# A2R-Lab/indy7-mpc

Measured on AMD Instinct MI355X. Metric: SQP-MPC solves/sec (Indy7 6-DOF, N=32), higher is better.
Workload: dtype f64

## Files before the change

indy7_mpc_amd/csrc/i7m_admm.h:

```cpp
#pragma once

#include "i7m_kernels.h"

namespace i7m {

struct AdmmCfg {
  double rho0, sigma, alpha, eps_abs, eps_rel, adapt_tol;
  int max_iter, check, scaling, gap, adapt_interval, pad;
};

struct AdmmArgs {
  SolveParams P;
  AdmmCfg A;
  const double* lin;
  const double* cost;
  const double* qpd;
  const double* xu;
  const double* xs;
  const int* active;
  double* sol;
  double *sx, *sz, *sy, *sq, *srho;
  double *Pq, *Pd, *I, *qs, *ls, *D, *E, *Dt, *Et, *R, *w;
  double* cs;
  int* iters;
  int* status;
  int sqp_iter;
  int b0;
  int ablate;
  const double* abase;
  long abytes;
};

constexpr int ADMM_FSTRIDE = 19;
constexpr int ADMM_SCALE_WPE = 2;
constexpr int ADMM_FACTOR_WPE = 2;
constexpr int ADM_REC = 300, REC_J = 180;
__device__ __forceinline__ int adm_lw(int i) { return i < 16 ? 2 * ((i + 2) / 2) : 18; }
__device__ __forceinline__ int adm_lrow(int i) {
  const int h = i >> 1;
  return i < 16 ? 2 * h * (h + 1) + (i & 1) * (2 * h + 2) : 144 + 18 * (i - 16);
}
__device__ __forceinline__ int adm_lrec(int i, int j) { return adm_lrow(i) + j; }
constexpr unsigned A5_OOB = 0x7ff00000u;
__device__ __forceinline__ __amdgpu_buffer_rsrc_t a4_rsrc(const void* base, long bytes) {
  const unsigned long long u = (unsigned long long)base;
  const unsigned lo = __builtin_amdgcn_readfirstlane((unsigned)u), hi = __builtin_amdgcn_readfirstlane((unsigned)(u >> 32));
  const int nb = __builtin_amdgcn_readfirstlane((int)bytes);
  return __builtin_amdgcn_make_buffer_rsrc((void*)(((unsigned long long)hi << 32) | lo), (short)0, nb, 0x00020000);
}
__device__ __forceinline__ void adm_stage_J(double* sJ, const double* Jc, int l) {
  for (int e = l; e < 216; e += 64) {
    const int i = e / 18, j = e - 18 * i;
    double v;
    if (i < 6) v = j == i ? Jc[i] : (j == 6 + i ? Jc[6 + i] : 0.0);
    else v = Jc[12 + 18 * (i - 6) + j];
    sJ[e] = v;
  }
}

template <int n>
__device__ __forceinline__ double adm_dot2(double init, const double* a, int sa, const double* b, int sb) {
  double av[n], bv[n];
#pragma unroll
  for (int i = 0; i < n; ++i) {
    av[i] = a[sa * i];
    bv[i] = b[sb * i];
  }
  double acc = init;
#pragma unroll
  for (int i = 0; i < n; ++i) acc += av[i] * bv[i];
  return acc;
}

template <int W>
__device__ __forceinline__ double adm_max(double v) {
#pragma unroll
  for (int off = W / 2; off >= 1; off >>= 1) v = fmax(v, __shfl_xor(v, off, W));
  return v;
}
template <int W>
__device__ __forceinline__ double adm_sum(double v) {
#pragma unroll
  for (int off = W / 2; off >= 1; off >>= 1) v += __shfl_xor(v, off, W);
  return v;
}
__device__ __forceinline__ double adm_wave_max(double v) { return adm_max<64>(v); }
__device__ __forceinline__ double adm_wave_sum(double v) { return adm_sum<64>(v); }
__device__ __forceinline__ double adm_limit(double v) { return v < 1e-4 ? 1.0 : (v > 1e4 ? 1e4 : v); }

__device__ __forceinline__ double adm_jk(const double* L, double dt, int i, int j) {
  if (i < 6) return j == i ? 1.0 : (j == 6 + i ? dt : 0.0);
  const int r = i - 6;
  return j < 6 ? L[6 * r + j] : (j < 12 ? L[36 + 6 * r + j - 6] : L[72 + 6 * r + j - 12]);
}

#define ADM_CHK_LOADS_FIRST()                          \
  do {                                                 \
    __builtin_amdgcn_sched_group_barrier(0x020, 24, 0); \
    __builtin_amdgcn_sched_group_barrier(0x002, 96, 0); \
  } while (0)

__device__ inline bool adm_check(const AdmmArgs& a, int N, int T, int m, double c, double rho, const double* x,
                                 const double* z, const double* y, const double* qs, const double* ls, const double* D,
                                 const double* E, const double* Jb, const double* Ib, const double* Pq, const double* Pd,
                                 double* rho_est, int l, double es = 1.0) {
  constexpr int W = 16;
  double pr = 0.0, zn = 0.0, an = 0.0, pri = 0.0, pn = 0.0;
  double dr = 0.0, qn = 0.0, atn = 0.0, pxn = 0.0, dua = 0.0, dn = 0.0, xPx = 0.0, qx = 0.0, sc = 0.0;
  for (int r = l; r < m; r += W) {
    const int k = r / 12, i = r - 12 * k;
    const int kk = k > 0 ? k - 1 : 0, iq = i < 6 ? i : 0, iv = i < 6 ? 0 : i - 6;
    const double* G = Jb + ADM_REC * kk;
    const double* xk = x + 18 * kk;
    const double* Gr = G + 12 + 18 * iv;
    const double ib = Ib[r], xr = x[18 * k + i], er = E[r], zr = z[r], yr = y[r], lr = ls[r];
    const double ga = G[iq], gb = G[6 + iq], xa = xk[iq], xb = xk[6 + iq];
    double gv[18], xv[18];
#pragma unroll
    for (int j = 0; j < 18; ++j) {
      gv[j] = Gr[j];
      xv[j] = xk[j];
    }
    ADM_CHK_LOADS_FIRST();
    double aq = 0.0, av = 0.0;
    aq += ga * xa;
    aq += gb * xb;
#pragma unroll
    for (int j = 0; j < 18; ++j) av += gv[j] * xv[j];
    const double acc = i < 6 ? aq : av;
    const double ax = k == 0 ? ib * xr : acc + ib * xr;
    const double ei = 1.0 / er;
    pr = fmax(pr, fabs(ei * (ax - zr)));
    zn = fmax(zn, fabs(ei * zr));
    an = fmax(an, fabs(ei * ax));
    pri = fmax(pri, fabs(ax - zr));
    pn = fmax(pn, fmax(fabs(zr), fabs(ax)));
    sc += lr * fmax(yr, 0.0) + lr * fmin(yr, 0.0);
  }
  for (int e = l; e < T; e += W) {
    const int k = e / 18, j = e - 18 * k;
    const int jq = j < 12 ? j : 0, jc = j < 6 ? j : 0, kc = k < N - 1 ? k : 0;
    const int jy = j < 6 ? j : (j < 12 ? j - 6 : 0);
    const double* G = Jb + ADM_REC * kc;
    const double* yk = y + 12 * (k < N - 1 ? k + 1 : 0);
    const double xe = x[e], de = D[e], qe = qs[e], pde = Pd[e], ibj = Ib[12 * k + jq], yj = y[12 * k + jq];
    const double gq = G[jq], yq = yk[jy];
    double pq[6], xq[6], gv[6], yv[6];
#pragma unroll
    for (int t = 0; t < 6; ++t) {
      pq[t] = Pq[36 * k + 6 * jc + t];
      xq[t] = x[18 * k + t];
      gv[t] = G[12 + 18 * t + j];
      yv[t] = yk[6 + t];
    }
    ADM_CHK_LOADS_FIRST();
    double pa = 0.0;
#pragma unroll
    for (int t = 0; t < 6; ++t) pa += pq[t] * xq[t];
    const double px = j < 6 ? pa : pde * xe;
    const double at0 = j < 12 ? ibj * yj : 0.0;
    double at1 = j < 12 ? at0 + gq * yq : at0;
#pragma unroll
    for (int t = 0; t < 6; ++t) at1 += gv[t] * yv[t];
    const double aty = k < N - 1 ? at1 : at0;
    const double di = 1.0 / de;
    dr = fmax(dr, fabs(di * ((qe + px) + aty)));
    qn = fmax(qn, fabs(di * qe));
    atn = fmax(atn, fabs(di * aty));
    pxn = fmax(pxn, fabs(di * px));
    dua = fmax(dua, fabs(qe + px + aty));
    dn = fmax(dn, fmax(fabs(qe), fmax(fabs(aty), fabs(px))));
    xPx += xe * px;
    qx += qe * xe;
  }
  pr = adm_max<W>(pr); zn = adm_max<W>(zn); an = adm_max<W>(an); pri = adm_max<W>(pri); pn = adm_max<W>(pn);
  dr = adm_max<W>(dr); qn = adm_max<W>(qn); atn = adm_max<W>(atn); pxn = adm_max<W>(pxn);
  dua = adm_max<W>(dua); dn = adm_max<W>(dn);
  xPx = adm_sum<W>(xPx); qx = adm_sum<W>(qx); sc = adm_sum<W>(sc);
  const double cinv = 1.0 / c;
  {
    const double p = pri / (pn + 1e-30), d = dua / (dn + 1e-30);
    double rn = rho * sqrt(p / (d + 1e-30));
    *rho_est = fmin(fmax(rn, 1e-6), 1e6);
  }
  dr *= cinv;
  const double ea = es * a.A.eps_abs, er = es * a.A.eps_rel;
  if (!(pr < ea + er * fmax(zn, an))) return false;
  if (!(dr < ea + er * cinv * fmax(qn, fmax(atn, pxn)))) return false;
  if (a.A.gap) {
    xPx *= cinv; qx *= cinv; sc *= cinv;
    const double gp = xPx + qx + sc;
    if (!(fabs(gp) < ea + er * fmax(fabs(xPx), fmax(fabs(qx), fabs(sc))))) return false;
  }
  return true;
}

__device__ __forceinline__ double adm_pq(const double* w, int i, int j) { return w[6] * (w[i] * w[j]); }
template <int CT>
__device__ __forceinline__ double adm_scale(const AdmmArgs& a, int b, int N, int T, int m, const double* LIN,
                                            const double* CO, const double* QD, const double* X, double* qold,
                                            double* Pq, double* Pd, double* Jb, double* Ib, double* qs, double* ls,
                                            double* D, double* E, double* sD, double* sE, double* sDt, double* sRM, int l) {
  constexpr int RT = 2 * CT / 3;
  const double dt = a.P.dt;
  double qv[CT], etv[RT], dtv[CT <= 9 ? CT : 1];
#pragma unroll
  for (int t = 0; t < CT; ++t) {
    const int e = l + 64 * t;
    qv[t] = 0.0;
    if (e < T) {
      sD[e] = 1.0;
      qv[t] = qold[e];
    }
  }
#pragma unroll
  for (int t = 0; t < RT; ++t)
    if (l + 64 * t < m) sE[l + 64 * t] = 1.0;
  wave_sync_fence();
  double c = 1.0;
  auto pcol = [&](const double* Cp, int k, int j, double dj) {
    const double* w = Cp + COST_STRIDE * k;
    const int jq = j < 6 ? j : 0;
    double mq = 0.0;
#pragma unroll
    for (int i = 0; i < 6; ++i) mq = fmax(mq, fabs(adm_pq(w, i, jq)) * (sD[18 * k + i] * dj) * c);
    const double pd = j < 12 ? w[7] : w[8];
    return j < 6 ? mq : fabs(pd) * (dj * dj) * c;
  };
  constexpr bool REG = CT <= 9;
  const int ks = l >> 1, hs = l & 1;
  const bool sv = REG && ks < N - 1;
  double av[REG ? 3 : 1][REG ? 18 : 1];
  if constexpr (REG) {
    const double* L = LIN + LIN_STRIDE * (sv ? ks : 0);
#pragma unroll
    for (int r = 0; r < 3; ++r)
#pragma unroll
      for (int j = 0; j < 18; ++j) {
        const int jb = j < 6 ? j : (j < 12 ? 30 + j : 60 + j);
        av[r][j] = sv ? L[jb + 6 * (3 * hs + r)] : 0.0;
      }
  }
#ifdef I7M_DIAG
  const int ss_p = a.ablate >= 300000 ? a.ablate - 300000 : -1;
  const bool ss_on = ss_p >= 0 && blockIdx.x == 0;
  unsigned long long ss_t[8] = {0, 0, 0, 0, 0, 0, 0, 0};
#endif
#define AS_STAMP(i) I7M_STAMP(ss_t, i, ss_on && pass == ss_p)
  for (int pass = 0; pass < a.A.scaling; ++pass) {
    AS_STAMP(0);
    const double* Lp = LIN;
    const double* Cp = CO;
    int lp = l;
    asm volatile("" : "+v"(lp));
    if constexpr (REG) {
      double cm[18];
#pragma unroll
      for (int j = 0; j < 18; ++j) cm[j] = 0.0;
      const int kq = sv ? ks : 0;
#pragma unroll
      for (int r = 0; r < 3; ++r) {
        const double er = sE[12 * (kq + 1) + 6 + 3 * hs + r];
        double rm = 0.0;
#pragma unroll
        for (int j = 0; j < 18; ++j) {
          const double pv = er * fabs(av[r][j]) * sD[18 * kq + j];
          rm = fmax(rm, pv);
          cm[j] = fmax(cm[j], pv);
        }
        if (sv) sRM[12 * (kq + 1) + 6 + 3 * hs + r] = rm;
      }
#pragma unroll
      for (int j = 0; j < 18; ++j) {
        const long long u = __double_as_longlong(cm[j]);
        const int lo = __builtin_amdgcn_update_dpp(0, (int)u, 0xB1, 0xf, 0xf, true);
// ... 349 lines not shown
```

indy7_mpc_amd/csrc/i7m_admm_iter.h:

```cpp
#pragma once

#include "i7m_admm.h"

namespace i7m {

constexpr int A5_LREC = 316, A5_LJ = 196;
__device__ __forceinline__ int a5_lrow(int i) {
  const int g = i >> 2;
  return i < 16 ? 8 * g * (g + 1) + 4 * (g + 1) * (i - 4 * g) : 160 + 18 * (i - 16);
}

constexpr int A5_RI = 10;
constexpr int A5_VI = 3;
constexpr int A5_VP = 42;
constexpr int A5_RP = A5_LREC / 2;
template <int n>
__device__ __forceinline__ double a4_bc(double v) {
  return __builtin_amdgcn_update_dpp(0.0, v, 0x150 + n, 0xf, 0xf, false);
}
__device__ __forceinline__ double a4_dpp32(double v, int ctrl_is_shl) {
  const long long u = __double_as_longlong(v);
  int lo = (int)u, hi = (int)(u >> 32);
  if (ctrl_is_shl) {
    lo = __builtin_amdgcn_update_dpp(lo, lo, 0x106, 0xf, 0xf, false);
// ... 111 lines not shown
  return {lo, b16, b17};
}
__device__ __forceinline__ A4Vec a4_ltmul(const A4CL& L, const A4CT& C, const A4Vec& v) {
  double lo = a4_dot16<2>(v.lo, C.Lt);
  lo = __fma_rn(L.Lc16, v.h16, lo);
  lo = __fma_rn(L.Lc17, v.h17, lo);
  return {lo, __fma_rn(L.d76, v.h17, __dmul_rn(L.d66, v.h16)), __dmul_rn(L.d77, v.h17)};
}
__device__ __forceinline__ A4Vec a4_jtmul(const A4CJ& C, double u, A4Vec init) {
  const double us = a4_shr6(u);
  const double lo = __dadd_rn(__fma_rn(C.Jd, us, init.lo), a4_dot6(u, C.Jt));
  return {lo, __dadd_rn(init.h16, a4_dot6(u, C.J16)), __dadd_rn(init.h17, a4_dot6(u, C.J17))};
}
__device__ __forceinline__ double a4_jmul(const A4CR& C, int c, const A4Vec& v) {
  double a = a4_dot16(v.lo, C.Jr);
  a = __fma_rn(C.Jr[16], v.h16, a);
  a = __fma_rn(C.Jr[17], v.h17, a);
  const double sp = __fma_rn(C.Jq1, a4_shl6(v.lo), __dmul_rn(C.Jq0, v.lo));
  return c < 6 ? sp : a;
}

typedef unsigned int a4u2 __attribute__((ext_vector_type(2)));
__device__ __forceinline__ double a5_ld(__amdgpu_buffer_rsrc_t r, unsigned off) {
  return __builtin_bit_cast(double, __builtin_amdgcn_raw_buffer_load_b64(r, off, 0, 0));
}
__device__ __forceinline__ void a5_st(double v, __amdgpu_buffer_rsrc_t r, unsigned off) {
  __builtin_amdgcn_raw_buffer_store_b64(__builtin_bit_cast(a4u2, v), r, off, 0, 0);
}
__device__ __forceinline__ unsigned a5_dma_off(int t) { return 1024u * (unsigned)(t & 3); }
__device__ __forceinline__ void a5_dma(__amdgpu_buffer_rsrc_t r, unsigned lds, const unsigned (&ro)[A5_RI], unsigned so,
                                       const unsigned (&vo)[A5_VI]) {
  unsigned keep;
  asm volatile(
      "s_mov_b32 %0, m0\n\t"
      "s_mov_b32 m0, %1\n\t"
      "s_nop 0\n\t"
      "buffer_load_dwordx4 %2, %15, %16 offen lds\n\t"
      "buffer_load_dwordx4 %3, %15, %16 offen offset:1024 lds\n\t"
      "buffer_load_dwordx4 %4, %15, %16 offen offset:2048 lds\n\t"
      "buffer_load_dwordx4 %5, %15, %16 offen offset:3072 lds\n\t"
      "s_add_u32 m0, m0, 0x1000\n\ts_nop 0\n\t"
      "buffer_load_dwordx4 %6, %15, %16 offen lds\n\t"
      "buffer_load_dwordx4 %7, %15, %16 offen offset:1024 lds\n\t"
      "buffer_load_dwordx4 %8, %15, %16 offen offset:2048 lds\n\t"
      "buffer_load_dwordx4 %9, %15, %16 offen offset:3072 lds\n\t"
      "s_add_u32 m0, m0, 0x1000\n\ts_nop 0\n\t"
      "buffer_load_dwordx4 %10, %15, %16 offen lds\n\t"
      "buffer_load_dwordx4 %11, %15, %16 offen offset:1024 lds\n\t"
      "buffer_load_dwordx4 %12, %15, 0 offen offset:2048 lds\n\t"
      "buffer_load_dwordx4 %13, %15, 0 offen offset:3072 lds\n\t"
      "s_add_u32 m0, m0, 0x1000\n\ts_nop 0\n\t"
      "buffer_load_dwordx4 %14, %15, 0 offen lds\n\t"
      "s_mov_b32 m0, %0"
      : "=&s"(keep)
      : "s"(__builtin_amdgcn_readfirstlane(lds)), "v"(ro[0]), "v"(ro[1]), "v"(ro[2]), "v"(ro[3]), "v"(ro[4]), "v"(ro[5]), "v"(ro[6]), "v"(ro[7]),
        "v"(ro[8]), "v"(ro[9]), "v"(vo[0]), "v"(vo[1]), "v"(vo[2]), "s"(r), "s"(__builtin_amdgcn_readfirstlane(so))
      : "memory");
}
__device__ __forceinline__ void a5_wait() { asm volatile("s_waitcnt vmcnt(13)" ::: "memory"); }
__device__ __forceinline__ void a5_dma2(__amdgpu_buffer_rsrc_t r, unsigned lds, const unsigned (&ro)[5], unsigned so,
                                        const unsigned (&vo)[2]) {
  unsigned keep;
  asm volatile(
      "s_mov_b32 %0, m0\n\t"
      "s_mov_b32 m0, %1\n\t"
      "s_nop 0\n\t"
      "buffer_load_dwordx4 %2, %9, %10 offen lds\n\t"
      "buffer_load_dwordx4 %3, %9, %10 offen offset:1024 lds\n\t"
      "buffer_load_dwordx4 %4, %9, %10 offen offset:2048 lds\n\t"
      "buffer_load_dwordx4 %5, %9, %10 offen offset:3072 lds\n\t"
      "s_add_u32 m0, m0, 0x1000\n\ts_nop 0\n\t"
      "buffer_load_dwordx4 %6, %9, %10 offen lds\n\t"
      "buffer_load_dwordx4 %7, %9, 0 offen offset:1024 lds\n\t"
      "buffer_load_dwordx4 %8, %9, 0 offen offset:2048 lds\n\t"
      "s_mov_b32 m0, %0"
      : "=&s"(keep)
      : "s"(__builtin_amdgcn_readfirstlane(lds)), "v"(ro[0]), "v"(ro[1]), "v"(ro[2]), "v"(ro[3]), "v"(ro[4]),
        "v"(vo[0]), "v"(vo[1]), "s"(r), "s"(__builtin_amdgcn_readfirstlane(so))
      : "memory");
}
__device__ __forceinline__ void a5_wait2() { asm volatile("s_waitcnt vmcnt(7)" ::: "memory"); }
__device__ __forceinline__ void a5_drain() { asm volatile("s_waitcnt vmcnt(0)" ::: "memory"); }

__device__ __forceinline__ bool a4_check(const AdmmArgs& a, int N, int T, int m, long bq, double c_cost, double rho,
                                         int c, double* rho_est, double es = 1.0) {
  return adm_check(a, N, T, m, c_cost, rho, a.sx + bq * T, a.sz + bq * m, a.sy + bq * m, a.qs + bq * T, a.ls + bq * m,
                   a.D + bq * T, a.E + bq * m, a.R + bq * N * ADM_REC + REC_J, a.I + bq * m, a.Pq + bq * N * 36,
                   a.Pd + bq * T, rho_est, c, es);
}
__device__ __forceinline__ int a4_closing_status(const AdmmArgs& a, int N, int T, int m, long bq, double c_cost,
                                                 double rho, int c, bool solved) {
  auto test = [&](double es) {
    double rest = rho;
    return a4_check(a, N, T, m, bq, c_cost, rho, c, &rest, es);
  };
  const bool last_checked = a.A.check && a.A.max_iter % a.A.check == 0;
  const bool exact = last_checked ? false : test(1.0);
  const bool approx = exact ? false : test(10.0);
  return solved ? 1 : (exact ? 1 : (approx ? 2 : 0));
}
__device__ __forceinline__ void a4_finish(const AdmmArgs& a, long b, bool lead, double rho, bool solved, int done_it,
                                          int status) {
  if (lead) {
    a.srho[b] = rho;
    if (a.iters) a.iters[b * 8 + a.sqp_iter] = solved ? done_it : a.A.max_iter;
    if (a.status) a.status[b * 8 + a.sqp_iter] = status;
  }
}
__device__ __forceinline__ void a4_solution(const AdmmArgs& a, long b, const double* x, int e0, int stride) {
  const int T = a.P.T;
  const double* D = a.D + b * T;
  double* sol = a.sol + b * T;
  for (int e = e0; e < T; e += stride) sol[e] = D[e] * x[e];
}

struct A5Stamps {
#ifdef I7M_DIAG
  unsigned long long t[9] = {0, 0, 0, 0, 0, 0, 0, 0, 0};
  int it, s;
  bool on = false;
  __device__ __forceinline__ explicit A5Stamps(int ablate)
      : it(ablate >= 100000 && ablate < 200000 && blockIdx.x == 0 ? (ablate - 100000) / 100 : -1), s(ablate % 100) {}
  __device__ __forceinline__ void step(int i, int st) { on = i == it && st == s; }
  __device__ __forceinline__ void write(int ablate, int layout) const {
    if (it >= 0) tl_write_stamps(t, 9, ablate, layout);
  }
#else
  __device__ __forceinline__ explicit A5Stamps(int) {}
  __device__ __forceinline__ void step(int, int) {}
  __device__ __forceinline__ void write(int, int) const {}
#endif
};
#define A5_STAMP(st, i) I7M_STAMP((st).t, i, (st).on)

struct A4K {
  int c;
  bool lo12;
  double rv, ri, sg, al, al1;
};
struct A4Op {
  double v0, v1, z1, y1, l1, ib1;
  double2 hv0, hv1;
};
struct A4Co {
  A4CJ J;
  A4CL L;
  A4CT T;
  A4CR Jr;
  const double* R;
};
struct A4Carry {
  A4Vec hc;
  double tk, ibk;
  double b0z, b0y, b0l, b0i, nx0;
  double2 nx0h;
};
struct A4New {
  double zn, yn, xn, xn16, xn17;
};
__device__ __forceinline__ double a4_t(const A4K& K, double z, double y) {
  return __dmul_rn(K.rv, __dsub_rn(z, __dmul_rn(K.ri, y)));
}
__device__ __forceinline__ void a4_coef_begin(A4Co& C, const double* R, int c) {
  C.R = R;
  a4_ldj(C.J, R, c);
  a4_ldl(C.L, R, R + a5_lrow(c), c);
}
template <int SB>
__device__ __forceinline__ A4Vec a4_llt(A4Co& C, const A4Vec& r, bool jr, int c, A5Stamps& st) {
  A5_STAMP(st, SB);
  a4_ldt(C.T, C.R, c);
  const A4Vec y = a4_lmul(C.L, r);
  A5_STAMP(st, SB + 1);
  if (jr) a4_ldr(C.Jr, C.R, c);
  const A4Vec o = a4_ltmul(C.L, C.T, y);
  A5_STAMP(st, SB + 2);
  return o;
}
template <int SB, class Put>
__device__ __forceinline__ void a4_forward(const A4K& K, const A4Op& o, A4Co& C, A4Carry& S, A5Stamps& st, Put&& put) {
  const double t1 = a4_t(K, o.z1, o.y1);
  const double init = K.lo12 ? __dmul_rn(S.ibk, S.tk) : 0.0;
  A4Vec r = a4_jtmul(C.J, t1, A4Vec{init, 0.0, 0.0});
  r.lo = __dadd_rn(__dsub_rn(__dmul_rn(K.sg, o.v0), o.v1), r.lo);
  r.h16 = __dadd_rn(__dsub_rn(__dmul_rn(K.sg, o.hv0.x), o.hv1.x), r.h16);
  r.h17 = __dadd_rn(__dsub_rn(__dmul_rn(K.sg, o.hv0.y), o.hv1.y), r.h17);
  const double rc = __dsub_rn(r.lo, __dmul_rn(__dmul_rn(K.rv, S.ibk), S.hc.lo));
  r.lo = K.lo12 ? rc : r.lo;
  const A4Vec h = a4_llt<SB>(C, r, true, K.c, st);
  put(h);
  A5_STAMP(st, SB + 3);
  S.hc.lo = a4_jmul(C.Jr, K.c, h);
  S.tk = t1;
  S.ibk = o.ib1;
  A5_STAMP(st, SB + 4);
}
template <int SB>
__device__ __forceinline__ void a4_forward_last(const A4K& K, const A4Op& o, A4Co& C, A4Carry& S, A5Stamps& st) {
  A4Vec r{K.lo12 ? __dmul_rn(S.ibk, S.tk) : 0.0, 0.0, 0.0};
  r.lo = __dadd_rn(__dsub_rn(__dmul_rn(K.sg, o.v0), o.v1), r.lo);
  r.lo = __dsub_rn(r.lo, __dmul_rn(__dmul_rn(K.rv, S.ibk), S.hc.lo));
  r.lo = K.lo12 ? r.lo : 0.0;
  S.hc = a4_llt<SB>(C, r, false, K.c, st);
}
__device__ __forceinline__ A4New a4_relax(const A4K& K, double zt, double z, double y, double l, const A4Vec& xt, double x,
                                          double x16, double x17) {
  const double zr = __dadd_rn(__dmul_rn(K.al, zt), __dmul_rn(K.al1, z));
  double zn = __dadd_rn(zr, __dmul_rn(K.ri, y));
  zn = fmin(fmax(zn, l), l);
  const double yn = __dadd_rn(y, __dmul_rn(K.rv, __dsub_rn(zr, zn)));
  const double xn = __dadd_rn(__dmul_rn(K.al, xt.lo), __dmul_rn(K.al1, x));
  const double xn16 = __dadd_rn(__dmul_rn(K.al, xt.h16), __dmul_rn(K.al1, x16));
  const double xn17 = __dadd_rn(__dmul_rn(K.al, xt.h17), __dmul_rn(K.al1, x17));
  return {zn, yn, xn, xn16, xn17};
}
template <int SB, class Put>
__device__ __forceinline__ void a4_backward(const A4K& K, const A4Op& o, A4Co& C, A4Carry& S, A5Stamps& st, Put&& put) {
  const double u = __dmul_rn(__dmul_rn(K.rv, o.ib1), S.hc.lo);
  const A4Vec s2 = a4_llt<SB>(C, a4_jtmul(C.J, u, A4Vec{0.0, 0.0, 0.0}), true, K.c, st);
  const A4Vec xt{__dsub_rn(o.v0, s2.lo), __dsub_rn(o.hv0.x, s2.h16), __dsub_rn(o.hv0.y, s2.h17)};
  const double zt = __dadd_rn(a4_jmul(C.Jr, K.c, xt), __dmul_rn(o.ib1, S.hc.lo));
  A5_STAMP(st, SB + 3);
  put(a4_relax(K, zt, o.z1, o.y1, o.l1, S.hc, o.v1, o.hv1.x, o.hv1.y));
  S.hc = xt;
  A5_STAMP(st, SB + 4);
}
template <class Put>
__device__ __forceinline__ void a4_block0(const A4K& K, A4Carry& S, Put&& put) {
  const double zt = __dmul_rn(S.b0i, S.hc.lo);
  const A4New n = a4_relax(K, zt, S.b0z, S.b0y, S.b0l, S.hc, S.nx0, S.nx0h.x, S.nx0h.y);
  put(n);
  S.nx0 = n.xn;
  S.nx0h = make_double2(n.xn16, n.xn17);
  S.b0z = n.zn;
  S.b0y = n.yn;
  S.tk = a4_t(K, n.zn, n.yn);
  S.ibk = S.b0i;
  S.hc = A4Vec{0.0, 0.0, 0.0};
}

template <bool ADAPT, int PW = 4>
__device__ __forceinline__ void admm_iter4(const AdmmArgs& a) {
  static_assert(PW == 4 || PW == 2, "four or two problems per wave");
  constexpr int RI = PW == 4 ? A5_RI : 5, VI = PW == 4 ? A5_VI : 2;
  constexpr int SLOT = 64 * (RI + VI), VD = 2 * 64 * RI;
  constexpr int PL = PW - 1;
  const SolveParams& P = a.P;
  const int N = P.N, T = P.T, m = 12 * N;
  const int l = threadIdx.x, p = l >> 4, c = l & 15;
  __shared__ double2 sRing[3 * SLOT];
  double* const ring = (double*)sRing;
  const unsigned ring_lds = (unsigned)(unsigned long)(__attribute__((address_space(3))) void*)sRing;
  const int bb = a.b0 + PW * (int)blockIdx.x;
  A5Stamps st(a.ablate);
  bool run = p < PW && bb + p < P.B && !(a.active && !a.active[bb + p]);
  const bool act = run;
  if (!__ballot(run)) return;
  const int bown = bb + (p < PW ? p : PL), bq = bown < P.B ? bown : bb;
  const auto rA = a4_rsrc(a.abase, a.abytes);
  auto boff = [&](const double* q) { return (unsigned)__builtin_amdgcn_readfirstlane((int)((const char*)q - (const char*)a.abase)); };
  const unsigned oX = boff(a.sx), oZ = boff(a.sz), oY = boff(a.sy), oQ = boff(a.qs), oL = boff(a.ls), oI = boff(a.I);
  const unsigned oH = boff(a.w), oR = boff(a.R);
  const unsigned xT = oX + 8u * (unsigned)(bown * T), hT = oH + 8u * (unsigned)(bown * T);
  const unsigned zM = oZ + 8u * (unsigned)(bown * m), yM = oY + 8u * (unsigned)(bown * m);
  const unsigned lM = oL + 8u * (unsigned)(bown * m), iM = oI + 8u * (unsigned)(bown * m);
  const double c_cost = a.cs[bq];
  double rho = a.srho[bq];
  A4K K{c, c < 12, 1e3 * rho, 1.0 / (1e3 * rho), a.A.sigma, a.A.alpha, 1.0 - a.A.alpha};
  const int cc = c < 12 ? c : 11;
  const int c16 = 16 + (c & 1);
  const bool lo12 = K.lo12, lo2 = c < 2;
  unsigned ro[RI], vF[VI], vB[VI], vD[VI], vZ[VI], vo[VI];
  int vcls[VI];
  auto offsets = [&]() {
    const unsigned long long rm = __ballot(run);
#pragma unroll
    for (int t = 0; t < RI; ++t) {
      const int g = 64 * t + l, q = g / A5_RP, j = g - A5_RP * q;
      const bool ok = q < PW && ((rm >> (16 * q)) & 1);
      int hp;
      if (j < 80) {
        int r = 0;
#pragma unroll
        for (int i = 1; i < 16; ++i) r = 2 * j >= a5_lrow(i) ? i : r;
        const int cp = 2 * j - a5_lrow(r);
        hp = cp < adm_lw(r) ? (adm_lrow(r) + cp) / 2 : -1;
      } else {
        hp = j - 8;
      }
      ro[t] = (ok && hp >= 0 ? oR + 8u * (unsigned)((bb + q) * N * ADM_REC) + 16u * hp : A5_OOB) - a5_dma_off(t);
    }
#pragma unroll
    for (int u = 0; u < VI; ++u) {
      const int g = 64 * u + l, q = g / A5_VP, j = g - A5_VP * q;
      const bool ok = q < PW && ((rm >> (16 * q)) & 1);
      const unsigned rT = 8u * (unsigned)((bb + q) * T), rM = 8u * (unsigned)((bb + q) * m);
      unsigned f, bk;
      int cl;
      if (j < 9) {
        f = oX + rT + 16u * j; bk = oH + rT + 16u * j; cl = 0;
      } else if (j < 18) {
        f = oQ + rT + 16u * (j - 9); bk = oX + rT + 16u * (j - 9); cl = 1;
      } else {
        const int jj = j - 18, w = jj / 6;
        f = (w == 0 ? oZ + 0u : w == 1 ? oY + 0u : w == 2 ? oL + 0u : oI + 0u) + rM + 16u * (jj - 6 * w);
        bk = f; cl = w == 0 ? 3 : 2;
      }
      const unsigned o = a5_dma_off(RI + u);
      vF[u] = (ok ? f : A5_OOB) - o;
      vB[u] = (ok ? bk : A5_OOB) - o;
      vD[u] = ok ? (cl < 2 ? 144u : 96u) : 0u;
      vZ[u] = ok && cl == 3 ? oL - oZ : 0u;
      vcls[u] = cl;
    }
  };
  offsets();
  auto vfull = [&](int s, bool zl) {
    const bool fwd = s < N;
    const int k = fwd ? s : 2 * N - 1 - s;
    const int k1 = k + 1 < N ? k + 1 : N - 1;
    const int kb = fwd ? k : k1;
#pragma unroll
    for (int u = 0; u < VI; ++u) {
      const unsigned st = vcls[u] == 0 ? 144u * k : (vcls[u] == 1 ? 144u * kb : 96u * k1);
      vo[u] = (fwd ? vF[u] + 0u : vB[u] + 0u) + (zl ? vZ[u] + st : st);
    }
  };
  auto issue = [&](int s, int slot, bool zl) {
    const bool fwd = s < N;
    const int k = fwd ? s : 2 * N - 1 - s;
    if (s == 0 || s == N - 1 || s == N || s == N + 1) {
// ... 42 lines not shown
    int sn = s + 2, sl = slot + 2;
    if (sn >= 2 * N) sn -= 2 * N;
    if (sl >= 3) sl -= 3;
    issue(sn, sl, it > 1 || sn < s);
    A5_STAMP(st, 2);
    const double* Sl = ring + 2 * SLOT * slot;
    const double* V = Sl + VD + 2 * A5_VP * (p < PW ? p : PL);
    o.v0 = V[ci];
    o.v1 = V[18 + cb];
    o.hv0 = make_double2(V[16], V[17]);
    o.hv1 = make_double2(V[34], V[35]);
    o.z1 = V[36 + cc];
    o.y1 = V[48 + cc];
    o.l1 = V[60 + cc];
    o.ib1 = V[72 + cc];
    a4_coef_begin(C, Sl + A5_LREC * (p < PW ? p : PL), c);
    A5_STAMP(st, 3);
  };
  auto so = [&](bool ok, unsigned off) { return run && ok ? off + 0u : A5_OOB + 0u; };
  auto fwd = [&](int k) {
    a4_forward<4>(K, o, C, S, st, [&](const A4Vec& h) {
      a5_st(h.lo, rA, so(true, hT + 8u * (18 * k + c)));
      a5_st(c == 0 ? h.h16 + 0.0 : h.h17 + 0.0, rA, so(lo2, hT + 8u * (18 * k + c16)));
    });
  };
  auto fwd_last = [&]() {
    a4_forward_last<4>(K, o, C, S, st);
    a5_st(S.hc.lo, rA, so(lo12, hT + 8u * (18 * (N - 1) + c)));
  };
  auto bwd = [&](int k) {
    a4_backward<4>(K, o, C, S, st, [&](const A4New& n) {
      const bool last1 = k + 1 == N - 1;
      const unsigned ob = 8u * (12 * (k + 1) + c);
      a5_st(n.zn, rA, so(lo12 && it == 1, zM + ob));
      a5_st(n.yn, rA, so(lo12, yM + ob));
      a5_st(n.xn, rA, so(!last1 || lo12, xT + 8u * (18 * (k + 1) + c)));
      a5_st(c == 0 ? n.xn16 + 0.0 : n.xn17 + 0.0, rA, so(!last1 && lo2, xT + 8u * (18 * (k + 1) + c16)));
      if (k == 0) {
        nx1 = n.xn;
        nx1h = make_double2(n.xn16, n.xn17);
        nz1 = n.zn;
        ny1 = n.yn;
      }
    });
  };
  int slot = 0;
  auto next = [&]() { slot = slot == 2 ? 0 : slot + 1; };
  for (; it <= a.A.max_iter; ++it) {
    for (int s = 0; s < N - 1; ++s) {
      begin(s, slot, c, c);
      if (it > 1 && s == 0) {
        o.v0 = S.nx0; o.hv0 = S.nx0h; o.z1 = nz1; o.y1 = ny1;
      }
      if (it > 1 && s == 1) {
        o.v0 = nx1; o.hv0 = nx1h;
      }
      fwd(s);
      next();
    }
    begin(N - 1, slot, cc, cc);
    if (it > 1 && N == 2) o.v0 = nx1;
    fwd_last();
    next();
    begin(N, slot, cc, cc);
    next();
    for (int s = N + 1; s < 2 * N; ++s) {
      begin(s, slot, c, s == N + 1 ? cc : c + 0);
      bwd(2 * N - 1 - s);
      next();
    }
    a4_block0(K, S, [&](const A4New& n) {
      a5_st(n.zn, rA, so(lo12 && it == 1, zM + 8u * c));
      a5_st(n.yn, rA, so(lo12, yM + 8u * c));
      a5_st(n.xn, rA, so(true, xT + 8u * c));
      a5_st(c == 0 ? n.xn16 + 0.0 : n.xn17 + 0.0, rA, so(lo2, xT + 8u * c16));
    });
    const bool chk = a.A.check && it % a.A.check == 0;
    const bool adapt = ADAPT && a.A.adapt_interval && it % a.A.adapt_interval == 0;
    if (chk || adapt) {
      a5_drain();
      __builtin_amdgcn_fence(__ATOMIC_RELEASE, "workgroup");
      __builtin_amdgcn_fence(__ATOMIC_ACQUIRE, "workgroup");
      double rest = rho;
      const bool ok = a4_check(a, N, T, m, bq, c_cost, rho, c, &rest);
      bool fin = false;
      if (chk && ok && run) {
        run = false;
        solved = true;
        done_it = it;
        fin = true;
      }
      bool reload = false;
      if constexpr (ADAPT) {
        const bool moved = run && adapt && (rest > rho * a.A.adapt_tol || rest < rho / a.A.adapt_tol);
        const unsigned long long mv = __ballot(moved);
        if (mv) {
          if (moved) {
            rho = rest;
            K.rv = 1e3 * rho;
            K.ri = 1.0 / K.rv;
          }
          for (int q = 0; q < PW; ++q) {
            if (!((mv >> (16 * q)) & 0xffff)) continue;
            const long bq2 = bb + q;
            const double rq = __shfl(rho, 16 * q, 64);
            double* scr = ring;
            adm_factor(a, N, rq, a.Pq + bq2 * N * 36, a.Pd + bq2 * T, a.I + bq2 * m, a.R + bq2 * N * ADM_REC, scr,
                       scr + 30 * ADMM_FSTRIDE + 388, scr + 30 * ADMM_FSTRIDE, scr + 18 * ADMM_FSTRIDE,
                       scr + 2048, l);
          }
          __builtin_amdgcn_fence(__ATOMIC_RELEASE, "workgroup");
          __builtin_amdgcn_fence(__ATOMIC_ACQUIRE, "workgroup");
          S.tk = a4_t(K, S.b0z, S.b0y);
          reload = true;
        }
      }
      if (!__ballot(run)) break;
      if (__ballot(fin)) {
        offsets();
        vfull(1, true);
      }
      if (reload) {
        slot = 0;
        issue(0, 0, true);
        issue(1, 1, true);
      }
    }
  }
  a5_drain();
  __builtin_amdgcn_fence(__ATOMIC_RELEASE, "workgroup");
  __builtin_amdgcn_fence(__ATOMIC_ACQUIRE, "workgroup");
  int st_v = solved ? 1 : 0;
  if (__ballot(act && !solved)) st_v = a4_closing_status(a, N, T, m, bq, c_cost, rho, c, solved);
  if (l == 0) st.write(a.ablate, 0);
  a4_finish(a, bown, c == 0 && act, rho, solved, done_it, st_v);
  if (act) a4_solution(a, bown, a.sx + (long)bown * T, c, 16);
}

constexpr int ARES_N = 32;
__device__ __forceinline__ void a5_dma1(__amdgpu_buffer_rsrc_t r, unsigned lds, unsigned off) {
  unsigned keep;
  asm volatile(
      "s_mov_b32 %0, m0\n\t"
      "s_mov_b32 m0, %1\n\t"
      "s_nop 0\n\t"
      "buffer_load_dwordx4 %2, %3, 0 offen lds\n\t"
      "s_mov_b32 m0, %0"
      : "=&s"(keep)
      : "s"(__builtin_amdgcn_readfirstlane(lds)), "v"(off), "s"(r)
      : "memory");
}
template <int NR>
__device__ __forceinline__ void admm_iter_res(const AdmmArgs& a) {
  const SolveParams& P = a.P;
  const int N = P.N, T = P.T, m = 12 * N;
  const int l = threadIdx.x, c = l & 15;
  const int b = a.b0 + (int)blockIdx.x;
  if (b >= P.B || (a.active && !a.active[b])) return;
  __shared__ double2 sRec2[NR * A5_LREC / 2];
  __shared__ double2 sV2[(3 * 18 + 4 * 12) * NR / 2 + 8];
  double* const sRec = (double*)sRec2;
  double* const sX = (double*)sV2;
  double* const sQ = sX + 18 * NR;
  double* const sH = sQ + 18 * NR;
  double* const sZ = sH + 18 * NR;
  double* const sY = sZ + 12 * NR;
  double* const sL = sY + 12 * NR;
  double* const sI = sL + 12 * NR;
  double* const sJunk = sI + 12 * NR;
  auto lds = [](const void* q) { return (unsigned)(unsigned long)(__attribute__((address_space(3))) const void*)q; };
  const auto rA = a4_rsrc(a.abase, a.abytes);
  auto boff = [&](const double* q) { return (unsigned)__builtin_amdgcn_readfirstlane((int)((const char*)q - (const char*)a.abase)); };
  const unsigned oX = boff(a.sx + (long)b * T), oQ = boff(a.qs + (long)b * T), oZ = boff(a.sz + (long)b * m);
  const unsigned oY = boff(a.sy + (long)b * m), oL = boff(a.ls + (long)b * m), oI = boff(a.I + (long)b * m);
  const unsigned oR = boff(a.R + (long)b * N * ADM_REC);
  {
    const int np = N * A5_RP;
    for (int g0 = 0; g0 < np; g0 += 64) {
      const int g = g0 + l, k = g / A5_RP, j = g - A5_RP * k;
      int hp;
      if (j < 80) {
        int r = 0;
#pragma unroll
        for (int i = 1; i < 16; ++i) r = 2 * j >= a5_lrow(i) ? i : r;
        const int cp = 2 * j - a5_lrow(r);
        hp = cp < adm_lw(r) ? (adm_lrow(r) + cp) / 2 : -1;
      } else {
        hp = j - 8;
      }
      a5_dma1(rA, lds(sRec) + 16u * g0, g < np && hp >= 0 ? oR + 8u * (unsigned)(k * ADM_REC) + 16u * hp : A5_OOB);
    }
    auto copy = [&](double* dst, unsigned src, int n) {
      for (int g0 = 0; g0 < n / 2; g0 += 64) a5_dma1(rA, lds(dst) + 16u * g0, g0 + l < n / 2 ? src + 16u * (g0 + l) : A5_OOB);
    };
    copy(sX, oX, T);
    copy(sQ, oQ, T);
    copy(sZ, oZ, m);
    copy(sY, oY, m);
    copy(sL, oL, m);
    copy(sI, oI, m);
    if (l < 6) {
      sX[T + l] = 0.0;
      sQ[T + l] = 0.0;
    }
    a5_drain();
    __builtin_amdgcn_fence(__ATOMIC_RELEASE, "workgroup");
    __builtin_amdgcn_fence(__ATOMIC_ACQUIRE, "workgroup");
  }
  auto flush = [&]() {
    for (int e = l; e < T; e += 64) a5_st(sX[e], rA, oX + 8u * e);
    for (int e = l; e < m; e += 64) {
      a5_st(sZ[e], rA, oZ + 8u * e);
      a5_st(sY[e], rA, oY + 8u * e);
    }
    a5_drain();
    __builtin_amdgcn_fence(__ATOMIC_RELEASE, "workgroup");
    __builtin_amdgcn_fence(__ATOMIC_ACQUIRE, "workgroup");
  };
  const double c_cost = a.cs[b];
  const double rho = a.srho[b];
  const A4K K{c, c < 12, 1e3 * rho, 1.0 / (1e3 * rho), a.A.sigma, a.A.alpha, 1.0 - a.A.alpha};
  const int cc = c < 12 ? c : 11;
  const bool lo12 = K.lo12, lo2 = c < 2;
  double* const junk = sJunk + c;
  int it = 1;
  A4Carry S;
  S.hc = A4Vec{0.0, 0.0, 0.0};
  S.b0z = sZ[cc];
  S.b0y = sY[cc];
  S.b0l = sL[cc];
  S.b0i = sI[cc];
  S.nx0 = sX[c];
  S.nx0h = make_double2(sX[16], sX[17]);
  S.tk = a4_t(K, S.b0z, S.b0y);
  S.ibk = S.b0i;
  double nz1 = 0.0;
  int done_it = 0;
  bool solved = false;
  A4Op o;
  A4Co C;
  A5Stamps st(a.ablate);
  auto begin = [&](int s, int k, const double* V0, const double* V1, int k1, int ci, int cb) {
    st.step(it, s);
    A5_STAMP(st, 0);
    o.v0 = V0[ci];
    o.v1 = V1[cb];
    o.hv0 = make_double2(V0[16], V0[17]);
    o.hv1 = make_double2(V1[16], V1[17]);
    o.z1 = (it > 1 ? sL : sZ)[12 * k1 + cc];
    o.y1 = sY[12 * k1 + cc];
    o.l1 = sL[12 * k1 + cc];
    o.ib1 = sI[12 * k1 + cc];
    a4_coef_begin(C, sRec + A5_LREC * k, c);
    A5_STAMP(st, 1);
  };
  for (; it <= a.A.max_iter; ++it) {
    for (int k = 0; k < N - 1; ++k) {
      begin(k, k, sX + 18 * k, sQ + 18 * k, k + 1, c, c);
      if (it > 1 && k == 0) o.z1 = nz1;
      a4_forward<2>(K, o, C, S, st, [&](const A4Vec& h) {
        double* const H = sH + 18 * k;
        H[c] = h.lo;
        *(lo2 ? H + 16 + c : junk) = c == 0 ? h.h16 : h.h17;
      });
    }
    begin(N - 1, N - 1, sX + 18 * (N - 1), sQ + 18 * (N - 1), N - 1, cc, cc);
    a4_forward_last<2>(K, o, C, S, st);
    for (int k = N - 2; k >= 0; --k) {
      const bool last1 = k + 1 == N - 1;
      begin(2 * N - 1 - k, k, sH + 18 * k, sX + 18 * (k + 1), k + 1, c, last1 ? cc : c);
      a4_backward<2>(K, o, C, S, st, [&](const A4New& n) {
        const int ob = 12 * (k + 1);
        *(lo12 && it == 1 ? sZ + ob + c : junk) = n.zn;
        *(lo12 ? sY + ob + c : junk) = n.yn;
        double* const X1 = sX + 18 * (k + 1);
        *(!last1 || lo12 ? X1 + c : junk) = n.xn;
        *(!last1 && lo2 ? X1 + 16 + c : junk) = c == 0 ? n.xn16 : n.xn17;
        if (k == 0) nz1 = n.zn;
      });
    }
    a4_block0(K, S, [&](const A4New& n) {
      *(lo12 && it == 1 ? sZ + c : junk) = n.zn;
      *(lo12 ? sY + c : junk) = n.yn;
      sX[c] = n.xn;
      *(lo2 ? sX + 16 + c : junk) = c == 0 ? n.xn16 : n.xn17;
    });
    if (a.A.check && it % a.A.check == 0) {
      flush();
      double rest = rho;
      if (a4_check(a, N, T, m, b, c_cost, rho, c, &rest)) {
        solved = true;
        done_it = it;
        break;
      }
    }
  }
  if (!solved) flush();
  int st_v = solved ? 1 : 0;
  if (!solved) st_v = a4_closing_status(a, N, T, m, b, c_cost, rho, c, false);
  if (l == 0) st.write(a.ablate, 1);
  a4_finish(a, b, l == 0, rho, solved, done_it, st_v);
  a4_solution(a, b, sX, l, 64);
}

template <bool ADAPT>
__global__ void __launch_bounds__(64) __attribute__((amdgpu_waves_per_eu(1, 1))) k_admm_iter(AdmmArgs a) {
  admm_iter4<ADAPT>(a);
}
__global__ void __launch_bounds__(64) __attribute__((amdgpu_waves_per_eu(2, 2))) k_admm_iter2(AdmmArgs a) {
  admm_iter4<false, 2>(a);
}
__global__ void __launch_bounds__(64) __attribute__((amdgpu_waves_per_eu(1, 1))) k_admm_iter_res(AdmmArgs a) {
  admm_iter_res<ARES_N>(a);
}
#undef A5_STAMP

}
```

Before: 401,300.

## Unroll convergence check, use DPP reductions, and read check inputs from LDS

The ADMM convergence check is unrolled across several rows and columns per lane so more loads are in flight, and its cross-lane max/sum reductions now use DPP row rotations in place of shuffles. The resident-solver variant runs the check directly on the LDS copies of x, z, y, q, l, I and the Jacobian records, so it no longer flushes state to global memory before every check, and flushes only once at the end. The solution write is also batched with explicit scheduling. The cost is higher register pressure from the unrolling, plus explicit FMA use that can slightly change rounding in the termination tests.

```diff
diff --git a/indy7_mpc_amd/csrc/i7m_admm.h b/indy7_mpc_amd/csrc/i7m_admm.h
--- a/indy7_mpc_amd/csrc/i7m_admm.h
+++ b/indy7_mpc_amd/csrc/i7m_admm.h
@@ -94,103 +94,160 @@
   return j < 6 ? L[6 * r + j] : (j < 12 ? L[36 + 6 * r + j - 6] : L[72 + 6 * r + j - 12]);
 }
 
-#define ADM_CHK_LOADS_FIRST()                          \
-  do {                                                 \
-    __builtin_amdgcn_sched_group_barrier(0x020, 24, 0); \
-    __builtin_amdgcn_sched_group_barrier(0x002, 96, 0); \
+#define ADM_CHK_LOADS_FIRST(U)                               \
+  do {                                                       \
+    __builtin_amdgcn_sched_group_barrier(0x020, 48 * (U), 0); \
+    __builtin_amdgcn_sched_group_barrier(0x100, 48 * (U), 0); \
+    __builtin_amdgcn_sched_group_barrier(0x002, 512, 0);      \
   } while (0)
 
-__device__ inline bool adm_check(const AdmmArgs& a, int N, int T, int m, double c, double rho, const double* x,
-                                 const double* z, const double* y, const double* qs, const double* ls, const double* D,
-                                 const double* E, const double* Jb, const double* Ib, const double* Pq, const double* Pd,
-                                 double* rho_est, int l, double es = 1.0) {
+template <int n>
+__device__ __forceinline__ double adm_ror16(double v) {
+  const long long u = __double_as_longlong(v);
+  const int lo = __builtin_amdgcn_update_dpp(0, (int)u, 0x120 + n, 0xf, 0xf, false);
+  const int hi = __builtin_amdgcn_update_dpp(0, (int)(u >> 32), 0x120 + n, 0xf, 0xf, false);
+  return __longlong_as_double(((long long)hi << 32) | (unsigned int)lo);
+}
+template <int n>
+__device__ __forceinline__ void adm_chk_level(double (&mx)[11], double (&sm)[3]) {
+#pragma clang fp contract(off)
+  double tm[11], ts[3];
+#pragma unroll
+  for (int i = 0; i < 11; ++i) tm[i] = adm_ror16<n>(mx[i]);
+#pragma unroll
+  for (int i = 0; i < 3; ++i) ts[i] = adm_ror16<n>(sm[i]);
+#pragma unroll
+  for (int i = 0; i < 11; ++i) mx[i] = fmax(mx[i], tm[i]);
+#pragma unroll
+  for (int i = 0; i < 3; ++i) sm[i] = sm[i] + ts[i];
+}
+
+template <int UR, int UC>
+__device__ __forceinline__ bool adm_check(const AdmmArgs& a, int N, int T, int m, double c, double rho, const double* x,
+                                          const double* z, const double* y, const double* qs, const double* ls,
+                                          const double* D, const double* E, const double* Jb, int js, const double* Ib,
+                                          const double* Pq, const double* Pd, double* rho_est, int l, double es = 1.0) {
+#pragma clang fp contract(off)
   constexpr int W = 16;
   double pr = 0.0, zn = 0.0, an = 0.0, pri = 0.0, pn = 0.0;
   double dr = 0.0, qn = 0.0, atn = 0.0, pxn = 0.0, dua = 0.0, dn = 0.0, xPx = 0.0, qx = 0.0, sc = 0.0;
-  for (int r = l; r < m; r += W) {
-    const int k = r / 12, i = r - 12 * k;
-    const int kk = k > 0 ? k - 1 : 0, iq = i < 6 ? i : 0, iv = i < 6 ? 0 : i - 6;
-    const double* G = Jb + ADM_REC * kk;
-    const double* xk = x + 18 * kk;
-    const double* Gr = G + 12 + 18 * iv;
-    const double ib = Ib[r], xr = x[18 * k + i], er = E[r], zr = z[r], yr = y[r], lr = ls[r];
-    const double ga = G[iq], gb = G[6 + iq], xa = xk[iq], xb = xk[6 + iq];
-    double gv[18], xv[18];
-#pragma unroll
-    for (int j = 0; j < 18; ++j) {
-      gv[j] = Gr[j];
-      xv[j] = xk[j];
-    }
-    ADM_CHK_LOADS_FIRST();
-    double aq = 0.0, av = 0.0;
-    aq += ga * xa;
-    aq += gb * xb;
-#pragma unroll
-    for (int j = 0; j < 18; ++j) av += gv[j] * xv[j];
-    const double acc = i < 6 ? aq : av;
-    const double ax = k == 0 ? ib * xr : acc + ib * xr;
-    const double ei = 1.0 / er;
-    pr = fmax(pr, fabs(ei * (ax - zr)));
-    zn = fmax(zn, fabs(ei * zr));
-    an = fmax(an, fabs(ei * ax));
-    pri = fmax(pri, fabs(ax - zr));
-    pn = fmax(pn, fmax(fabs(zr), fabs(ax)));
-    sc += lr * fmax(yr, 0.0) + lr * fmin(yr, 0.0);
-  }
-  for (int e = l; e < T; e += W) {
-    const int k = e / 18, j = e - 18 * k;
-    const int jq = j < 12 ? j : 0, jc = j < 6 ? j : 0, kc = k < N - 1 ? k : 0;
-    const int jy = j < 6 ? j : (j < 12 ? j - 6 : 0);
-    const double* G = Jb + ADM_REC * kc;
-    const double* yk = y + 12 * (k < N - 1 ? k + 1 : 0);
-    const double xe = x[e], de = D[e], qe = qs[e], pde = Pd[e], ibj = Ib[12 * k + jq], yj = y[12 * k + jq];
-    const double gq = G[jq], yq = yk[jy];
-    double pq[6], xq[6], gv[6], yv[6];
-#pragma unroll
-    for (int t = 0; t < 6; ++t) {
-      pq[t] = Pq[36 * k + 6 * jc + t];
-      xq[t] = x[18 * k + t];
-      gv[t] = G[12 + 18 * t + j];
-      yv[t] = yk[6 + t];
-    }
-    ADM_CHK_LOADS_FIRST();
-    double pa = 0.0;
-#pragma unroll
-    for (int t = 0; t < 6; ++t) pa += pq[t] * xq[t];
-    const double px = j < 6 ? pa : pde * xe;
-    const double at0 = j < 12 ? ibj * yj : 0.0;
-    double at1 = j < 12 ? at0 + gq * yq : at0;
-#pragma unroll
-    for (int t = 0; t < 6; ++t) at1 += gv[t] * yv[t];
-    const double aty = k < N - 1 ? at1 : at0;
-    const double di = 1.0 / de;
-    dr = fmax(dr, fabs(di * ((qe + px) + aty)));
-    qn = fmax(qn, fabs(di * qe));
-    atn = fmax(atn, fabs(di * aty));
-    pxn = fmax(pxn, fabs(di * px));
-    dua = fmax(dua, fabs(qe + px + aty));
-    dn = fmax(dn, fmax(fabs(qe), fmax(fabs(aty), fabs(px))));
-    xPx += xe * px;
-    qx += qe * xe;
-  }
-  pr = adm_max<W>(pr); zn = adm_max<W>(zn); an = adm_max<W>(an); pri = adm_max<W>(pri); pn = adm_max<W>(pn);
-  dr = adm_max<W>(dr); qn = adm_max<W>(qn); atn = adm_max<W>(atn); pxn = adm_max<W>(pxn);
-  dua = adm_max<W>(dua); dn = adm_max<W>(dn);
-  xPx = adm_sum<W>(xPx); qx = adm_sum<W>(qx); sc = adm_sum<W>(sc);
+  for (int t0 = 0; t0 < m; t0 += W * UR) {
+    bool ok[UR], first[UR], qrow[UR];
+    double ib[UR], xr[UR], er[UR], zr[UR], yr[UR], lr[UR], ga[UR], gb[UR], xa[UR], xb[UR], gv[UR][18], xv[UR][18];
+#pragma unroll
+    for (int u = 0; u < UR; ++u) {
+      const int rr = t0 + W * u + l;
+      ok[u] = rr < m;
+      const int r = ok[u] ? rr : m - 1, k = r / 12, i = r - 12 * k;
+      first[u] = k == 0;
+      qrow[u] = i < 6;
+      const int kk = k > 0 ? k - 1 : 0, iq = i < 6 ? i : 0, iv = i < 6 ? 0 : i - 6;
+      const double* G = Jb + js * kk;
+      const double* xk = x + 18 * kk;
+      const double* Gr = G + 12 + 18 * iv;
+      ib[u] = Ib[r]; xr[u] = x[18 * k + i]; er[u] = E[r]; zr[u] = z[r]; yr[u] = y[r]; lr[u] = ls[r];
+      ga[u] = G[iq]; gb[u] = G[6 + iq]; xa[u] = xk[iq]; xb[u] = xk[6 + iq];
+#pragma unroll
+      for (int j = 0; j < 18; ++j) {
+        gv[u][j] = Gr[j];
+        xv[u][j] = xk[j];
+      }
+    }
+    ADM_CHK_LOADS_FIRST(UR);
+#pragma unroll
+    for (int u = 0; u < UR; ++u) {
+      double aq = __builtin_fma(ga[u], xa[u], 0.0);
+      aq = __builtin_fma(gb[u], xb[u], aq);
+      double av = 0.0;
+#pragma unroll
+      for (int j = 0; j < 18; ++j) av = __builtin_fma(gv[u][j], xv[u][j], av);
+      const double acc = qrow[u] ? aq : av;
+      const double ax = first[u] ? ib[u] * xr[u] : __builtin_fma(ib[u], xr[u], acc);
+      const double ei = 1.0 / er[u];
+      const double d = ax - zr[u];
+      const double t = __builtin_fma(lr[u], fmax(yr[u], 0.0), lr[u] * fmin(yr[u], 0.0));
+      pr = ok[u] ? fmax(pr, fabs(ei * d)) : pr;
+      zn = ok[u] ? fmax(zn, fabs(ei * zr[u])) : zn;
+      an = ok[u] ? fmax(an, fabs(ei * ax)) : an;
+      pri = ok[u] ? fmax(pri, fabs(d)) : pri;
+      pn = ok[u] ? fmax(pn, fmax(fabs(zr[u]), fabs(ax))) : pn;
+      sc = ok[u] ? sc + t : sc;
+    }
+  }
+  for (int t0 = 0; t0 < T; t0 += W * UC) {
+    bool ok[UC], j6[UC], j12[UC], notlast[UC];
+    double xe[UC], de[UC], qe[UC], pde[UC], ibj[UC], yj[UC], gq[UC], yq[UC], pq[UC][6], xq[UC][6], gv[UC][6], yv[UC][6];
+#pragma unroll
+    for (int u = 0; u < UC; ++u) {
+      const int ee = t0 + W * u + l;
+      ok[u] = ee < T;
+      const int e = ok[u] ? ee : T - 1, k = e / 18, j = e - 18 * k;
+      j6[u] = j < 6;
+      j12[u] = j < 12;
+      notlast[u] = k < N - 1;
+      const int jq = j < 12 ? j : 0, jc = j < 6 ? j : 0, kc = k < N - 1 ? k : 0;
+      const int jy = j < 6 ? j : (j < 12 ? j - 6 : 0);
+      const double* G = Jb + js * kc;
+      const double* yk = y + 12 * (k < N - 1 ? k + 1 : 0);
+      xe[u] = x[e]; de[u] = D[e]; qe[u] = qs[e]; pde[u] = Pd[e]; ibj[u] = Ib[12 * k + jq]; yj[u] = y[12 * k + jq];
+      gq[u] = G[jq]; yq[u] = yk[jy];
+#pragma unroll
+      for (int t = 0; t < 6; ++t) {
+        pq[u][t] = Pq[36 * k + 6 * jc + t];
+        xq[u][t] = x[18 * k + t];
+        gv[u][t] = G[12 + 18 * t + j];
+        yv[u][t] = yk[6 + t];
+      }
+    }
+    ADM_CHK_LOADS_FIRST(UC);
+#pragma unroll
+    for (int u = 0; u < UC; ++u) {
+      double pa = 0.0;
+#pragma unroll
+      for (int t = 0; t < 6; ++t) pa = __builtin_fma(pq[u][t], xq[u][t], pa);
+      const double px = j6[u] ? pa : pde[u] * xe[u];
+      const double iy = ibj[u] * yj[u];
+      const double at0 = j12[u] ? iy : 0.0;
+      double at1 = j12[u] ? __builtin_fma(gq[u], yq[u], iy) : 0.0;
+#pragma unroll
+      for (int t = 0; t < 6; ++t) at1 = __builtin_fma(gv[u][t], yv[u][t], at1);
+      const double aty = notlast[u] ? at1 : at0;
+      const double di = 1.0 / de[u];
+      const double s = (qe[u] + px) + aty;
+      dr = ok[u] ? fmax(dr, fabs(di * s)) : dr;
+      qn = ok[u] ? fmax(qn, fabs(di * qe[u])) : qn;
+      atn = ok[u] ? fmax(atn, fabs(di * aty)) : atn;
+      pxn = ok[u] ? fmax(pxn, fabs(di * px)) : pxn;
+      dua = ok[u] ? fmax(dua, fabs(s)) : dua;
+      dn = ok[u] ? fmax(dn, fmax(fabs(qe[u]), fmax(fabs(aty), fabs(px)))) : dn;
+      xPx = ok[u] ? __builtin_fma(xe[u], px, xPx) : xPx;
+      qx = ok[u] ? __builtin_fma(qe[u], xe[u], qx) : qx;
+    }
+  }
+  {
+    double mx[11] = {pr, zn, an, pri, pn, dr, qn, atn, pxn, dua, dn}, sm[3] = {xPx, qx, sc};
+    adm_chk_level<8>(mx, sm);
+    adm_chk_level<4>(mx, sm);
+    adm_chk_level<2>(mx, sm);
+    adm_chk_level<1>(mx, sm);
+    pr = mx[0]; zn = mx[1]; an = mx[2]; pri = mx[3]; pn = mx[4]; dr = mx[5]; qn = mx[6]; atn = mx[7]; pxn = mx[8];
+    dua = mx[9]; dn = mx[10];
+    xPx = sm[0]; qx = sm[1]; sc = sm[2];
+  }
   const double cinv = 1.0 / c;
   {
     const double p = pri / (pn + 1e-30), d = dua / (dn + 1e-30);
     double rn = rho * sqrt(p / (d + 1e-30));
     *rho_est = fmin(fmax(rn, 1e-6), 1e6);
   }
-  dr *= cinv;
+  dr = dr * cinv;
   const double ea = es * a.A.eps_abs, er = es * a.A.eps_rel;
-  if (!(pr < ea + er * fmax(zn, an))) return false;
-  if (!(dr < ea + er * cinv * fmax(qn, fmax(atn, pxn)))) return false;
+  if (!(pr < __builtin_fma(er, fmax(zn, an), ea))) return false;
+  if (!(dr < __builtin_fma(er * cinv, fmax(qn, fmax(atn, pxn)), ea))) return false;
   if (a.A.gap) {
-    xPx *= cinv; qx *= cinv; sc *= cinv;
-    const double gp = xPx + qx + sc;
-    if (!(fabs(gp) < ea + er * fmax(fabs(xPx), fmax(fabs(qx), fabs(sc))))) return false;
+    const double xs = cinv * xPx, qs1 = cinv * qx, ss = cinv * sc;
+    const double gp = __builtin_fma(cinv, sc, __builtin_fma(cinv, xPx, qs1));
+    if (!(fabs(gp) < __builtin_fma(er, fmax(fabs(xs), fmax(fabs(qs1), fabs(ss))), ea))) return false;
   }
   return true;
 }
diff --git a/indy7_mpc_amd/csrc/i7m_admm_iter.h b/indy7_mpc_amd/csrc/i7m_admm_iter.h
--- a/indy7_mpc_amd/csrc/i7m_admm_iter.h
+++ b/indy7_mpc_amd/csrc/i7m_admm_iter.h
@@ -217,17 +217,26 @@
 __device__ __forceinline__ void a5_wait2() { asm volatile("s_waitcnt vmcnt(7)" ::: "memory"); }
 __device__ __forceinline__ void a5_drain() { asm volatile("s_waitcnt vmcnt(0)" ::: "memory"); }
 
-__device__ __forceinline__ bool a4_check(const AdmmArgs& a, int N, int T, int m, long bq, double c_cost, double rho,
-                                         int c, double* rho_est, double es = 1.0) {
-  return adm_check(a, N, T, m, c_cost, rho, a.sx + bq * T, a.sz + bq * m, a.sy + bq * m, a.qs + bq * T, a.ls + bq * m,
-                   a.D + bq * T, a.E + bq * m, a.R + bq * N * ADM_REC + REC_J, a.I + bq * m, a.Pq + bq * N * 36,
-                   a.Pd + bq * T, rho_est, c, es);
-}
-__device__ __forceinline__ int a4_closing_status(const AdmmArgs& a, int N, int T, int m, long bq, double c_cost,
-                                                 double rho, int c, bool solved) {
+struct A4Src {
+  const double *x, *z, *y, *q, *l, *I, *J;
+  int js;
+};
+__device__ __forceinline__ A4Src a4_src_global(const AdmmArgs& a, int N, int T, int m, long bq) {
+  return {a.sx + bq * T, a.sz + bq * m, a.sy + bq * m, a.qs + bq * T, a.ls + bq * m, a.I + bq * m,
+          a.R + bq * N * ADM_REC + REC_J, ADM_REC};
+}
+template <int UR, int UC>
+__device__ __forceinline__ bool a4_check(const AdmmArgs& a, int N, int T, int m, long bq, const A4Src& s, double c_cost,
+                                         double rho, int c, double* rho_est, double es = 1.0) {
+  return adm_check<UR, UC>(a, N, T, m, c_cost, rho, s.x, s.z, s.y, s.q, s.l, a.D + bq * T, a.E + bq * m, s.J, s.js, s.I,
+                           a.Pq + bq * N * 36, a.Pd + bq * T, rho_est, c, es);
+}
+template <int UR, int UC>
+__device__ __forceinline__ int a4_closing_status(const AdmmArgs& a, int N, int T, int m, long bq, const A4Src& s,
+                                                 double c_cost, double rho, int c, bool solved) {
   auto test = [&](double es) {
     double rest = rho;
-    return a4_check(a, N, T, m, bq, c_cost, rho, c, &rest, es);
+    return a4_check<UR, UC>(a, N, T, m, bq, s, c_cost, rho, c, &rest, es);
   };
   const bool last_checked = a.A.check && a.A.max_iter % a.A.check == 0;
   const bool exact = last_checked ? false : test(1.0);
@@ -243,10 +252,28 @@
   }
 }
 __device__ __forceinline__ void a4_solution(const AdmmArgs& a, long b, const double* x, int e0, int stride) {
+  constexpr int G = 8;
   const int T = a.P.T;
   const double* D = a.D + b * T;
   double* sol = a.sol + b * T;
-  for (int e = e0; e < T; e += stride) sol[e] = D[e] * x[e];
+  for (int t0 = 0; t0 < T; t0 += G * stride) {
+    double d[G], v[G];
+#pragma unroll
+    for (int g = 0; g < G; ++g) {
+      const int e = t0 + g * stride + e0, ec = e < T ? e : T - 1;
+      d[g] = D[ec];
+      v[g] = x[ec];
+    }
+    __builtin_amdgcn_sched_group_barrier(0x020, 2 * G, 0);
+    __builtin_amdgcn_sched_group_barrier(0x100, G, 0);
+    __builtin_amdgcn_sched_group_barrier(0x002, G, 0);
+    __builtin_amdgcn_sched_group_barrier(0x040, G, 0);
+#pragma unroll
+    for (int g = 0; g < G; ++g) {
+      const int e = t0 + g * stride + e0;
+      if (e < T) sol[e] = d[g] * v[g];
+    }
+  }
 }
 
 struct A5Stamps {
@@ -382,6 +409,7 @@
   constexpr int PL = PW - 1;
   const SolveParams& P = a.P;
   const int N = P.N, T = P.T, m = 12 * N;
+  constexpr int UR = PW == 4 ? 3 : 1, UC = PW == 4 ? 4 : 2;
   const int l = threadIdx.x, p = l >> 4, c = l & 15;
   __shared__ double2 sRing[3 * SLOT];
   double* const ring = (double*)sRing;
@@ -590,7 +618,7 @@
       __builtin_amdgcn_fence(__ATOMIC_RELEASE, "workgroup");
       __builtin_amdgcn_fence(__ATOMIC_ACQUIRE, "workgroup");
       double rest = rho;
-      const bool ok = a4_check(a, N, T, m, bq, c_cost, rho, c, &rest);
+      const bool ok = a4_check<UR, UC>(a, N, T, m, bq, a4_src_global(a, N, T, m, bq), c_cost, rho, c, &rest);
       bool fin = false;
       if (chk && ok && run) {
         run = false;
@@ -639,7 +667,8 @@
   __builtin_amdgcn_fence(__ATOMIC_RELEASE, "workgroup");
   __builtin_amdgcn_fence(__ATOMIC_ACQUIRE, "workgroup");
   int st_v = solved ? 1 : 0;
-  if (__ballot(act && !solved)) st_v = a4_closing_status(a, N, T, m, bq, c_cost, rho, c, solved);
+  if (__ballot(act && !solved))
+    st_v = a4_closing_status<UR, UC>(a, N, T, m, bq, a4_src_global(a, N, T, m, bq), c_cost, rho, c, solved);
   if (l == 0) st.write(a.ablate, 0);
   a4_finish(a, bown, c == 0 && act, rho, solved, done_it, st_v);
   if (act) a4_solution(a, bown, a.sx + (long)bown * T, c, 16);
@@ -715,6 +744,8 @@
     __builtin_amdgcn_fence(__ATOMIC_RELEASE, "workgroup");
     __builtin_amdgcn_fence(__ATOMIC_ACQUIRE, "workgroup");
   }
+  constexpr int UR = 3, UC = 4;
+  const A4Src src{sX, sZ, sY, sQ, sL, sI, sRec + A5_LJ, A5_LREC};
   auto flush = [&]() {
     for (int e = l; e < T; e += 64) a5_st(sX[e], rA, oX + 8u * e);
     for (int e = l; e < m; e += 64) {
@@ -794,18 +825,17 @@
       *(lo2 ? sX + 16 + c : junk) = c == 0 ? n.xn16 : n.xn17;
     });
     if (a.A.check && it % a.A.check == 0) {
-      flush();
       double rest = rho;
-      if (a4_check(a, N, T, m, b, c_cost, rho, c, &rest)) {
+      if (a4_check<UR, UC>(a, N, T, m, b, src, c_cost, rho, c, &rest)) {
         solved = true;
         done_it = it;
         break;
       }
     }
   }
-  if (!solved) flush();
   int st_v = solved ? 1 : 0;
-  if (!solved) st_v = a4_closing_status(a, N, T, m, b, c_cost, rho, c, false);
+  if (!solved) st_v = a4_closing_status<UR, UC>(a, N, T, m, b, src, c_cost, rho, c, false);
+  flush();
   if (l == 0) st.write(a.ablate, 1);
   a4_finish(a, b, l == 0, rho, solved, done_it, st_v);
   a4_solution(a, b, sX, l, 64);
```

Result: no change. 403,900, median of 6 (+0.6%).
